# JokerYan/MS-GS

Hardware: AMD Instinct MI355X
Metric: Mpixels/s fwd+bwd @1080p, 1M Gaussians; fraction of HBM roofline (higher is better)
Workload: dtype f32

## Files before the change

__graft_entry__.py:

```python
import os
import subprocess
import sys

ROOT = os.path.dirname(os.path.abspath(__file__))
PKG = os.path.join(ROOT, "ms-gs_amd")


def _paths():
    for p in (ROOT, PKG, os.path.join(PKG, "host"), os.path.join(ROOT, "tests")):
        if p not in sys.path:
            sys.path.insert(0, p)


def build():
    subprocess.check_call(["make", "-C", PKG, "-j4"])
    subprocess.call(["make", "-C", PKG, "isa"], stdout=subprocess.DEVNULL, stderr=subprocess.DEVNULL)
    subprocess.check_call(["make", "-C", os.path.join(ROOT, "oracle")])
    _paths()
    import diff_gaussian_rasterization
    import gaussian_renderer
    import view_parallel
    lib = os.path.join(PKG, "lib", "libmsgs_hip.so")
    assert os.path.exists(lib), lib
    harness = os.path.join(PKG, "build", "libmsgs_sort_harness.so")
    assert os.path.exists(harness), harness
    harness = os.path.join(PKG, "build", "libmsgs_depth_sort_harness.so")
    assert os.path.exists(harness), harness
    print("built", lib)


def smoke():
    _paths()
    import torch
    assert torch.cuda.is_available(), "smoke() needs a GPU"
    import scenes
    from oracle import oracle_ctypes as oc
    from parity_utils import check_backward, check_forward, hip_render, small_scene
    torch.cuda.set_device(0)
    W, H = 160, 96
    sc, cam = small_scene(4000, W, H, seed=123, multiscale=True, scale_k=0.004 * 1920.0 / W * 0.25)
    st = dict(filter_small=True, filter_large=True, fade_size=0.0)
    bg = torch.tensor([0.1, 0.2, 0.3])
    dL = scenes.grad_seed(W, H, 123)
    out, pc, m2 = hip_render(sc, cam, st, bg, dL, device="cuda:0")
    orc = oc.rasterize(pc.seen, cam, st, bg)
    og = oc.backward(orc, dL)
    fwd = check_forward(out, orc, "smoke")
    bwd = check_backward(pc, m2, og, "smoke", flagged=orc.borderline_gaussians)
    print(f"smoke ok: visible={(out['radii'] > 0).sum().item()} fwd_maxdiff={fwd:.2e} bwd_rel={max(bwd.values()):.2e}")
# ... 7 lines not shown
```

ms-gs_amd/csrc/api.hip:

```cpp
#include "msgs_internal.h"

#include <atomic>
#include <new>

#include <cstring>

using namespace msgs;

namespace {

struct Timer {
    const msgs_timing_t* t;
    hipStream_t s;
    void begin(int k) const { if (t && t->ev[2 * k]) (void)hipEventRecord((hipEvent_t)t->ev[2 * k], s); }
    void end(int k) const { if (t && t->ev[2 * k + 1]) (void)hipEventRecord((hipEvent_t)t->ev[2 * k + 1], s); }
};

inline int check_inputs(const msgs_view_t* v, const msgs_gaussians_t* g) {
    if (!v || !g) return MSGS_ERR_INVALID_ARG;
    if (g->P < 0 || v->image_width <= 0 || v->image_height <= 0) return MSGS_ERR_INVALID_ARG;
    if (!v->bg || !v->viewmatrix || !v->projmatrix || !v->campos) return MSGS_ERR_INVALID_ARG;
    if (g->P > 0 && (!g->means3D || !g->opacities)) return MSGS_ERR_INVALID_ARG;
    if (g->raw_params) {
        if (g->raw_params != 1 && g->raw_params != 2) return MSGS_ERR_INVALID_ARG;
// ... 185 lines not shown
    ZeroJob zj1{nullptr, 0, (uint32_t*)(geom + GL.slab_hdr), (GL.occ_hdr - GL.slab_hdr) / 4 + sizeof(OccHeader) / 4 + 2 * (size_t)OCC_BUCKETS};
    const bool sort1_buckets = depth_sort_uses_buckets(P);
    const bool sort1_prezeroed = sort1_buckets ? depth_sort_zero_region(P, scratch + SL.sort, &zj1.p0, &zj1.n0)
                                               : radix_sort_zero_region(P, 0, 32, scratch + SL.sort, &zj1.p0, &zj1.n0);
    const bool occlusion = get_occlusion() != 0;
    uint32_t* heavy_list = occlusion ? (uint32_t*)(scratch + SL.heavy_list) : nullptr;
    uint32_t* heavy_count = occlusion ? (uint32_t*)(scratch + SL.heavy_count) : nullptr;
    uint32_t* heavy_blk = occlusion ? (uint32_t*)(scratch + SL.heavy_blk) : nullptr;
    tm.begin(MSGS_K_PREPROCESS);
    HIP_TRY(launch_preprocess(vp, *g, radii, pixel_sizes, geom, s, zj1, heavy_list, heavy_count, heavy_blk, g_deterministic.load() != 0));
    if (occlusion)
        HIP_TRY(launch_occlusion(vp, P, geom, heavy_list, heavy_count, heavy_blk, (OccCand*)(scratch + SL.occ_cand), s));
    tm.end(MSGS_K_PREPROCESS);
    if ((rc = debug_sync(view, s))) return rc;

    if (!blocking_sync()) sb.ensure();
    const bool polled = !blocking_sync() && sb.host != nullptr;
    const uint64_t ticket = ++sb.ticket;
    uint64_t* total_dev = (uint64_t*)(scratch + SL.total_out);
    uint64_t* status_dev = total_dev + 2;
    uint32_t* clamped_dev = (uint32_t*)(total_dev + 5);
    uint32_t* heavy_q_word = spec ? (uint32_t*)((char*)spec->buf.scratch2 + Stage2Scratch(spec->capacity).heavy_q) : nullptr;

    tm.begin(MSGS_K_DEPTH_SORT);
    if (sort1_buckets)
        HIP_TRY(depth_sort_buckets((const uint32_t*)(geom + GL.key), (uint32_t*)(geom + GL.skey), (uint32_t*)(geom + GL.order), P,
                                   scratch + SL.sort, s, sort1_prezeroed, (uint32_t*)(geom + GL.nvalid),
                                   (uint32_t*)(geom + GL.slab_hdr + DEPTH_SORT_INFO_OFFSET)));
    else
        HIP_TRY(radix_sort_pairs((uint32_t*)(geom + GL.key), nullptr, (uint32_t*)(geom + GL.skey),
                                 (uint32_t*)(geom + GL.order), P, 0, 32, scratch + SL.sort, s, sort1_prezeroed,
                                 (uint32_t*)(geom + GL.nvalid)));
    tm.end(MSGS_K_DEPTH_SORT);
    if ((rc = debug_sync(view, s))) return rc;
    tm.begin(MSGS_K_SCAN);
    HIP_TRY(exclusive_scan_u32((const uint32_t*)(geom + GL.tiles), (const uint32_t*)(geom + GL.order),
                               (uint32_t*)(geom + GL.offs), P, (uint64_t*)(scratch + SL.scan_partials), total_dev, s,
                               status_dev, polled ? sb.dev : nullptr, ticket,
                               (const uint32_t*)(geom + GL.nvalid), spec ? clamped_dev : nullptr,
                               spec ? (uint64_t)spec->capacity : 0, (const uint32_t*)(geom + GL.occ_hdr), heavy_q_word, nullptr,
                               vp.cell_sx >= 0 ? TILE_COUNT_MASK : 0xFFFFFFFFu,
                               vp.cell_sx >= 0 && slab_wanted(view, g) ? (uint32_t*)(geom + GL.offs_b) : nullptr,
                               &reinterpret_cast<SlabHeader*>(geom + GL.slab_hdr)->pad[0]));
    tm.end(MSGS_K_SCAN);
    pend.active = true;
    pend.polled = polled;
    pend.stream = s;
    pend.ticket = ticket;
    pend.host = sb.host;
    pend.status_dev = status_dev;
    if (spec)
        spec->launched_rc = forward_stage2_impl(view, g, geom_v, geom_bytes, spec->capacity, spec->buf, timing, stream,
                                                clamped_dev, polled ? sb.dev : nullptr, ticket);
    return MSGS_OK;
}

int forward_stage1_wait(PendingCount& pend, int64_t* num_instances_host) {
    *num_instances_host = 0;
    if (!pend.active) { t_last_info = 0; for (int k = 0; k < 4; ++k) t_last_feedback[k] = 0; return MSGS_OK; }
    pend.active = false;
    hipStream_t s = pend.stream;
    uint64_t host_status[3] = {0, 0, 0};
    if (pend.polled) {
        volatile uint64_t* hv = pend.host;
        const uint64_t ticket = pend.ticket;
        uint64_t spins = 0;
// ... 1296 lines not shown
```

ms-gs_amd/csrc/msgs_internal.h:

```cpp
#pragma once
#include <hip/hip_runtime.h>
#include <stdint.h>
#include <cmath>
#include <type_traits>
#include "../../include/msgs.h"

namespace msgs {

constexpr int TILE = MSGS_TILE;
constexpr int WAVE = 64;

struct __attribute__((aligned(16))) GaussRec { float4 r0, r1, r2; };

struct __attribute__((aligned(32))) BinRec { float4 q0, q1; };

#if defined(MSGS_GRAD_REC_F32)
typedef float grad_acc_t;
constexpr int GRAD_REC_FLOATS = 12;
#else
typedef double grad_acc_t;
constexpr int GRAD_REC_FLOATS = 10;
#endif
constexpr uint32_t TILE_ORDER_MAGIC = 0x4C505431u;
constexpr size_t GRAD_REC_BYTES = sizeof(grad_acc_t) * GRAD_REC_FLOATS;
// ... 122 lines not shown
static_assert(DEPTH_BIN_LO + DEPTH_BINS - 1 == (0x7F7FFFFFu >> DEPTH_BIN_SHIFT), "the top bin is the one of FLT_MAX");
constexpr int DEPTH_BUCKETS = 255;
constexpr int DEPTH_LDS_THREADS = 1024;
constexpr int DEPTH_LDS_ITEMS = 8;
constexpr int DEPTH_LDS_CAP = DEPTH_LDS_THREADS * DEPTH_LDS_ITEMS;
constexpr int64_t DEPTH_BUCKET_MAX_P = 1'500'000;
constexpr size_t DEPTH_SORT_INFO_OFFSET = 64;

__host__ __device__ inline uint32_t depth_bin(uint32_t key) {
    uint32_t b = key >> DEPTH_BIN_SHIFT;
    b = b < DEPTH_BIN_LO ? DEPTH_BIN_LO : b;
    b -= DEPTH_BIN_LO;
    return b < (uint32_t)DEPTH_BINS ? b : (uint32_t)DEPTH_BINS - 1u;
}

constexpr int DEPTH_HIST_KEYS = 32768;
constexpr int DEPTH_HIST_MAX_BLOCKS = 64;
constexpr int64_t DEPTH_BUCKET_HARD_MAX = (int64_t)DEPTH_HIST_KEYS * DEPTH_HIST_MAX_BLOCKS;
__host__ __device__ inline int depth_hist_blocks(int64_t n) {
    const int64_t b = (n + DEPTH_HIST_KEYS - 1) / DEPTH_HIST_KEYS;
    return b < 1 ? 1 : (b > DEPTH_HIST_MAX_BLOCKS ? DEPTH_HIST_MAX_BLOCKS : (int)b);
}

struct DepthSortScratch {
    size_t sort, coarse, map, bases, slices, total;
    __host__ __device__ explicit DepthSortScratch(int64_t n) {
        size_t o = 0;
        sort = o;   o = align256(o + SortScratch(n).total);
        coarse = o; o = align256(o + 4 * (size_t)DEPTH_COARSE);
        map = o;    o = align256(o + (size_t)DEPTH_BINS);
        bases = o;  o = align256(o + 4 * (size_t)(DEPTH_BUCKETS + 2 + 2));
        slices = o; o = align256(o + 2 * (size_t)DEPTH_BINS * depth_hist_blocks(n));
        total = o;
    }
    __host__ __device__ size_t zero_end() const { return coarse + 4 * (size_t)DEPTH_COARSE; }
};

struct Stage1Scratch {
    size_t sort, scan_partials, total_out, heavy_list, heavy_count, heavy_blk, occ_cand, total;
    __host__ __device__ explicit Stage1Scratch(int64_t P) {
        size_t o = 0;
        const size_t Pn = (size_t)(P > 0 ? P : 1);
        const size_t waves = 4 * ((Pn + 255) / 256);
        sort = o;          o = align256(o + DepthSortScratch(P).total);
        scan_partials = o; o = align256(o + 8 * (size_t)(scan_blocks(P > 0 ? P : 1) + 2));
        total_out = o;     o = align256(o + 64);
        heavy_list = o;    o = align256(o + 8 * 64 * waves);
        heavy_count = o;   o = align256(o + 4 * waves);
        heavy_blk = o;     o = align256(o + 2 * waves);
        occ_cand = o;      o = align256(o + sizeof(OccCand) * OCC_MAX_CAND);
        total = o;
    }
};

constexpr int DTRAV_SLOTS = 64;
struct BinningLayout {
    size_t ids, ranges, dtrav, total;
    __host__ __device__ BinningLayout(int64_t D, int64_t tiles) {
// ... 316 lines not shown
                                      const char* geom, const grad_acc_t* grad_rec, const msgs_grads_t& grads,
                                      hipStream_t s, bool textbook = false, bool depth = false,
                                      const CameraGrads* camera = nullptr);
hipError_t launch_blend_forward_literal(const ViewParams& vp, const char* geom, int P, const uint32_t* ids, const uint2* ranges,
                                        float* out_color, float* out_ps, float* out_depth, float* final_T, uint32_t* n_contrib,
                                        uint32_t* order_flag, hipStream_t s);
hipError_t launch_blend_backward_literal(const ViewParams& vp, const char* geom, int P, const uint32_t* ids, const uint2* ranges,
                                         const float* final_T, const uint32_t* n_contrib, const float* dL_dcolor, double* inst_grad,
                                         hipStream_t s, const float* dL_ddepth = nullptr,
                                         const float* dL_dalpha = nullptr);
hipError_t launch_sh_grad_from_views(int P, int n_views, int deg, const float* means3D, const float* campos,
                                     int64_t campos_stride, const float* drgb, int64_t drgb_stride, float scale,
                                     float* d_dc, float* d_rest, hipStream_t s);
hipError_t launch_mark_visible(int P, const float* means3D, const float* viewmatrix, const float* projmatrix,
                               uint8_t* present, hipStream_t s);
hipError_t radix_sort_pairs(uint32_t* keys_in, uint32_t* vals_in, uint32_t* keys_out, uint32_t* vals_out,
                            int64_t n, int begin_bit, int end_bit, char* scratch ,
                            hipStream_t s, bool pre_zeroed = false, uint32_t* n_valid_dev = nullptr,
                            const uint32_t* n_dev = nullptr, bool keys16 = false);
bool radix_sort_keys16_ok(int64_t n, int begin_bit, int end_bit);
bool radix_sort_zero_region(int64_t n, int begin_bit, int end_bit, char* scratch, uint32_t** ptr, size_t* words);
bool radix_sort_supports_device_count(int64_t n, int begin_bit, int end_bit);

hipError_t depth_sort_buckets(const uint32_t* keys_in, uint32_t* keys_out, uint32_t* vals_out, int64_t n,
                              char* scratch , hipStream_t s, bool pre_zeroed, uint32_t* n_valid_dev,
                              uint32_t* info = nullptr);
bool depth_sort_zero_region(int64_t n, char* scratch, uint32_t** ptr, size_t* words);
bool depth_sort_uses_buckets(int64_t n);
int set_depth_sort(int mode);
int get_depth_sort();

hipError_t exclusive_scan_u32(const uint32_t* in, const uint32_t* gather, uint32_t* out, int64_t n,
                              uint64_t* partials , uint64_t* total, hipStream_t s,
                              uint64_t* status = nullptr, uint64_t* host_mapped = nullptr, uint64_t ticket = 0,
                              const uint32_t* n_ptr = nullptr, uint32_t* clamped_total = nullptr, uint64_t clamp = 0,
                              const uint32_t* extra = nullptr,
                              uint32_t* zero_word = nullptr,
                              uint32_t* overflow_flag = nullptr, uint32_t in_mask = 0xFFFFFFFFu, uint32_t* side_out = nullptr,
                              uint32_t* side_flag = nullptr);
template <class F>
inline void with_bool(bool b, F&& f) {
    if (b) f(std::true_type{}); else f(std::false_type{});
}
hipError_t launch_zero(void* ptr, size_t bytes, hipStream_t s);
hipError_t launch_emit(const ViewParams& vp, int P, const char* geom, uint32_t* keys, uint32_t* ids,
                       int64_t D, hipStream_t s, ZeroJob zj = ZeroJob{nullptr, 0, nullptr, 0}, const uint32_t* D_dev = nullptr,
                       bool keys16 = false, uint32_t* heavy_q = nullptr, int slab = 0, const uint32_t* open_bits = nullptr,
                       int64_t density_D = 0);
hipError_t launch_slab_split(int P, char* geom, int64_t D, const uint32_t* D_dev, float fraction, uint32_t* open_bits,
// ... 140 lines not shown
```

ms-gs_amd/csrc/sort.hip:

```cpp
#include "msgs_internal.h"

#include <algorithm>
#include <atomic>
#include <cstdlib>

namespace msgs {

namespace {

__device__ __forceinline__ uint32_t wave_inclusive_scan(uint32_t v, int lane) {
#pragma unroll
    for (int off = 1; off < 64; off <<= 1) {
        const uint32_t n = (uint32_t)__shfl_up((int)v, off);
        if (lane >= off) v += n;
    }
    return v;
}

__device__ __forceinline__ uint32_t block_exclusive_scan(uint32_t v, uint32_t* s_wave , uint32_t* total) {
    const int lane = threadIdx.x & 63, w = threadIdx.x >> 6;
    const uint32_t inc = wave_inclusive_scan(v, lane);
    if (lane == 63) s_wave[w] = inc;
    __syncthreads();
    uint32_t base = 0;
// ... 51 lines not shown
    const int64_t base = (int64_t)blockIdx.x * SCAN_CHUNK + (int64_t)threadIdx.x * SCAN_ITEMS;
    uint32_t v[SCAN_ITEMS];
    if (gather) {
        uint32_t g[SCAN_ITEMS];
        scan_load_items(gather, base, n, g);
#pragma unroll
        for (int k = 0; k < SCAN_ITEMS; ++k) v[k] = base + k < n ? in[g[k]] : 0u;
        if (side_out) {
#pragma unroll
            for (int k = 0; k < SCAN_ITEMS; ++k) g[k] = v[k] >> TILE_COUNT_BITS;
            scan_store_items(side_out, base, n, g);
        }
#pragma unroll
        for (int k = 0; k < SCAN_ITEMS; ++k) v[k] &= in_mask;
        if (staged) scan_store_items(staged, base, n, v);
    } else {
        scan_load_items(in, base, n, v);
    }
    uint64_t sum = 0;
#pragma unroll
    for (int k = 0; k < SCAN_ITEMS; ++k) sum += v[k];
    const uint64_t total = block_sum_u64(sum, s_sum);
    if (threadIdx.x == 0) partials[blockIdx.x] = total;
}

__global__ __launch_bounds__(SCAN_THREADS) void scan_apply_fused_kernel(const uint32_t* in, uint32_t* out, int64_t n,
                                                                        const uint64_t* __restrict__ partials, int64_t nb,
                                                                        const uint32_t* __restrict__ n_ptr,
                                                                        uint64_t* __restrict__ total_out,
                                                                        uint64_t* __restrict__ status,
                                                                        volatile uint64_t* host, uint64_t ticket,
                                                                        uint32_t* __restrict__ clamped_total, uint64_t clamp,
                                                                        const uint32_t* __restrict__ extra,
                                                                        uint32_t* __restrict__ zero_word,
                                                                        uint32_t* __restrict__ overflow_flag) {
    __shared__ uint32_t s_wave[4];
    __shared__ uint64_t s_sum[4];
    if (n_ptr) n = (int64_t)*n_ptr;
    const int64_t chunk0 = (int64_t)blockIdx.x * SCAN_CHUNK;
    if (blockIdx.x != 0 && chunk0 >= n) return;
    const int64_t upto = blockIdx.x == 0 ? nb : (int64_t)blockIdx.x;
    uint64_t acc = 0;
    for (int64_t q = threadIdx.x; q < upto; q += SCAN_THREADS) acc += partials[q];
    const uint64_t sum = block_sum_u64(acc, s_sum);
    uint64_t base = sum;
    if (blockIdx.x == 0) {
        base = 0;
        if (threadIdx.x == 0) {
            if (total_out) *total_out = sum;
            if (zero_word) *zero_word = 0u;
            if (clamped_total) *clamped_total = (uint32_t)(sum < clamp ? sum : clamp);
            if (overflow_flag && sum > clamp) *overflow_flag = 1u;
            const uint64_t info = extra ? ((uint64_t)extra[0] | ((uint64_t)extra[1] << 32)) : 0ull;
            if (status) { status[0] = sum; status[1] = 0; status[2] = info; }
            if (host) {
                host[0] = sum;
                host[1] = 0;
                host[3] = info;
                __threadfence_system();
                host[2] = ticket;
            }
        }
        if (chunk0 >= n) return;
    }
    const int64_t tb = chunk0 + (int64_t)threadIdx.x * SCAN_ITEMS;
    uint32_t v[SCAN_ITEMS];
    scan_load_items(in, tb, n, v);
    uint32_t tsum = 0;
#pragma unroll
    for (int k = 0; k < SCAN_ITEMS; ++k) tsum += v[k];
    uint32_t total;
    uint32_t run = block_exclusive_scan(tsum, s_wave, &total) + (uint32_t)base;
#pragma unroll
    for (int k = 0; k < SCAN_ITEMS; ++k) {
        const uint32_t x = v[k];
        v[k] = run;
        run += x;
    }
    scan_store_items(out, tb, n, v);
}

struct ShiftDigit {
    int shift;
    uint32_t mask;
    __device__ __forceinline__ uint32_t operator()(uint32_t k) const { return (k >> shift) & mask; }
};
struct BucketDigit {
    const uint8_t* __restrict__ map;
    __device__ __forceinline__ uint32_t operator()(uint32_t k) const { return map[depth_bin(k)]; }
};

template <int ITEMS = SORT_ITEMS>
__device__ __forceinline__ int64_t elem_index(int64_t chunk_base, int w, int r, int lane) {
    return chunk_base + (int64_t)w * (64 * ITEMS) + r * 64 + lane;
}

template <int ITEMS, bool DROP = false, typename KeyT = uint32_t, typename Digit = ShiftDigit>
__global__ __launch_bounds__(SORT_THREADS) void radix_hist_kernel(const KeyT* __restrict__ keys, int64_t n,
                                                                  Digit dg, int64_t nblocks,
                                                                  uint32_t* __restrict__ hist,
                                                                  uint32_t* __restrict__ gsum, int gsize, int ngroups,
                                                                  const uint32_t* __restrict__ n_ptr = nullptr) {
    __shared__ uint32_t s_hist[256];
    const int64_t chunk_base = (int64_t)blockIdx.x * (SORT_THREADS * ITEMS);
    if (n_ptr) {
        n = (int64_t)*n_ptr;
        if (chunk_base >= n) return;
    }
    s_hist[threadIdx.x] = 0;
    __syncthreads();
    const int lane = threadIdx.x & 63, w = threadIdx.x >> 6;
    constexpr int KPV = 16 / (int)sizeof(KeyT);
    if (ITEMS % KPV == 0 && chunk_base + (int64_t)SORT_THREADS * ITEMS <= n) {
        const uint4* kv = reinterpret_cast<const uint4*>(keys + chunk_base);
#pragma unroll
        for (int r = 0; r < ITEMS / KPV; ++r) {
            const uint4 v = kv[r * SORT_THREADS + threadIdx.x];
            const uint32_t w4[4] = {v.x, v.y, v.z, v.w};
#pragma unroll
            for (int j = 0; j < KPV; ++j) {
                const uint32_t k = sizeof(KeyT) == 4 ? w4[j] : ((w4[j >> 1] >> ((j & 1) * 16)) & 0xFFFFu);
                if (!DROP || k != 0xFFFFFFFFu) atomicAdd(&s_hist[dg(k)], 1u);
            }
        }
    } else {
#pragma unroll
        for (int r = 0; r < ITEMS; ++r) {
            const int64_t i = elem_index<ITEMS>(chunk_base, w, r, lane);
            if (i < n) {
                const uint32_t k = (uint32_t)keys[i];
                if (!DROP || k != 0xFFFFFFFFu) atomicAdd(&s_hist[dg(k)], 1u);
            }
        }
    }
    __syncthreads();
    const uint32_t c = s_hist[threadIdx.x];
    hist[(int64_t)blockIdx.x * 256 + threadIdx.x] = c;
    if (c) atomicAdd(&gsum[(int64_t)(blockIdx.x / gsize) * 256 + threadIdx.x], c);
}

__global__ __launch_bounds__(256) void group_scan_kernel(uint32_t* __restrict__ gsum, int ngroups,
                                                         uint32_t* __restrict__ hist, int gsize, int64_t nblocks,
                                                         const uint32_t* __restrict__ n_ptr, int chunk) {
    if (n_ptr) {
        const int64_t n = (int64_t)*n_ptr;
        nblocks = (n + chunk - 1) / chunk;
        ngroups = (int)((nblocks + gsize - 1) / gsize);
        if ((int)blockIdx.x > ngroups) return;
        if (nblocks == 0) return;
    }
    const int d = threadIdx.x;
    if ((int)blockIdx.x < ngroups) {
        const int64_t first = (int64_t)blockIdx.x * gsize;
        const int rows = (int)min((int64_t)gsize, nblocks - first);
        uint32_t* q = hist + first * 256 + d;
        uint32_t run = 0;
#pragma unroll 8
        for (int k = 0; k < rows; ++k) {
            const uint32_t v = q[(int64_t)k * 256];
            q[(int64_t)k * 256] = run;
            run += v;
// ... 393 lines not shown
            if (valid && before == 0) s_cnt[w][d] = prev + (uint32_t)__popcll(peers);
        }
    }
    __syncthreads();
    uint32_t c[DEPTH_LDS_WAVES], ltot = 0;
    if (tid < 256) {
#pragma unroll
        for (int k = 0; k < DEPTH_LDS_WAVES; ++k) { c[k] = s_cnt[k][tid]; ltot += c[k]; }
    }
    const uint32_t inc = wave_inclusive_scan(ltot, lane);
    if (tid < 256 && lane == 63) s_wsum[w] = inc;
    __syncthreads();
    if (tid < 256) {
        uint32_t run = inc - ltot;
#pragma unroll
        for (int k = 0; k < 4; ++k) run += k < w ? s_wsum[k] : 0u;
#pragma unroll
        for (int k = 0; k < DEPTH_LDS_WAVES; ++k) { s_cnt[k][tid] = run; run += c[k]; }
        s_dcount[tid] = ltot;
    }
    __syncthreads();
}

__global__ __launch_bounds__(DEPTH_LDS_THREADS) void depth_lds_sort_kernel(uint32_t* keys_a, uint32_t* vals_a, uint32_t* keys_out,
                                                                           uint32_t* vals_out, const uint32_t* __restrict__ bases,
                                                                           int64_t n, uint32_t* __restrict__ info) {
    __shared__ uint32_t s_key[DEPTH_LDS_CAP], s_val[DEPTH_LDS_CAP];
    __shared__ uint32_t s_cnt[DEPTH_LDS_WAVES][256];
    __shared__ uint32_t s_wsum[4], s_dcount[256], s_run[256], s_or;
    const int tid = threadIdx.x, lane = tid & 63, w = tid >> 6;
    uint32_t lo = bases[blockIdx.x], hi = bases[blockIdx.x + 1];
    if (hi > (uint32_t)n) hi = (uint32_t)n;
    if (lo >= hi) return;
    const int64_t count = (int64_t)hi - lo;

    uint32_t key[DEPTH_LDS_ITEMS], val[DEPTH_LDS_ITEMS], rank[DEPTH_LDS_ITEMS];
    const bool fits = count <= DEPTH_LDS_CAP;
    const int R = fits ? ((int)count + DEPTH_LDS_THREADS - 1) / DEPTH_LDS_THREADS : DEPTH_LDS_ITEMS;

    if (tid == 0) s_or = 0;
    __syncthreads();
    {
        const uint32_t k0 = keys_a[lo];
        uint32_t diff = 0;
        if (fits) {
#pragma unroll
            for (int r = 0; r < DEPTH_LDS_ITEMS; ++r) {
                const int e = w * 64 * R + r * 64 + lane;
                const bool valid = r < R && e < (int)count;
                key[r] = valid ? keys_a[lo + e] : 0xFFFFFFFFu;
                val[r] = valid ? vals_a[lo + e] : 0u;
            }
#pragma unroll
            for (int r = 0; r < DEPTH_LDS_ITEMS; ++r) {
                const int e = w * 64 * R + r * 64 + lane;
                if (r < R && e < (int)count) diff |= key[r] ^ k0;
            }
        } else {
            for (int64_t i = tid; i < count; i += DEPTH_LDS_THREADS) diff |= keys_a[lo + i] ^ k0;
        }
        for (int off = 32; off > 0; off >>= 1) diff |= (uint32_t)__shfl_xor((int)diff, off);
        if (lane == 0 && diff) atomicOr(&s_or, diff);
    }
    __syncthreads();
    const int bits = 32 - __clz((int)s_or);
    int npass = (bits + 7) / 8;

    if (fits) {
        const int nloc = (int)count;
        if (npass == 0) {
#pragma unroll
            for (int r = 0; r < DEPTH_LDS_ITEMS; ++r) {
                const int e = w * 64 * R + r * 64 + lane;
                if (r < R && e < nloc) { keys_out[lo + e] = key[r]; vals_out[lo + e] = val[r]; }
            }
            return;
        }
        for (int p = 0; p < npass; ++p) {
            lds_rank(key, rank, R, nloc, 8 * p, s_cnt, s_wsum, s_dcount);
#pragma unroll
            for (int r = 0; r < DEPTH_LDS_ITEMS; ++r) {
                const int e = w * 64 * R + r * 64 + lane;
                if (r < R && e < nloc) {
                    const uint32_t lp = s_cnt[w][(key[r] >> (8 * p)) & 255u] + rank[r];
                    s_key[lp] = key[r];
                    s_val[lp] = val[r];
                }
            }
            __syncthreads();
            if (p + 1 < npass) {
#pragma unroll
                for (int r = 0; r < DEPTH_LDS_ITEMS; ++r) {
                    const int e = w * 64 * R + r * 64 + lane;
                    if (r < R && e < nloc) { key[r] = s_key[e]; val[r] = s_val[e]; }
                }
            }
        }
        for (int i = tid; i < nloc; i += DEPTH_LDS_THREADS) {
            keys_out[lo + i] = s_key[i];
            vals_out[lo + i] = s_val[i];
        }
        return;
    }

    if (tid == 0) atomicAdd(&info[1], 1u);
    if ((npass & 1) == 0) ++npass;
    for (int p = 0; p < npass; ++p) {
        const int shift = 8 * p;
        const uint32_t* src_k = (p & 1) ? keys_out : keys_a;
        const uint32_t* src_v = (p & 1) ? vals_out : vals_a;
        uint32_t* dst_k = (p & 1) ? keys_a : keys_out;
        uint32_t* dst_v = (p & 1) ? vals_a : vals_out;
        if (tid < 256) s_run[tid] = 0;
        __syncthreads();
        for (int64_t i = tid; i < count; i += DEPTH_LDS_THREADS)
            atomicAdd(&s_run[shift < 32 ? (src_k[lo + i] >> shift) & 255u : 0u], 1u);
        __syncthreads();
        if (tid == 0) {
            uint32_t run = 0;
            for (int d = 0; d < 256; ++d) { const uint32_t c = s_run[d]; s_run[d] = run; run += c; }
        }
        __syncthreads();
        for (int64_t c0 = 0; c0 < count; c0 += DEPTH_LDS_CAP) {
            const int nloc = (int)(count - c0 < DEPTH_LDS_CAP ? count - c0 : DEPTH_LDS_CAP);
// ... 2 lines not shown
            for (int r = 0; r < DEPTH_LDS_ITEMS; ++r) {
                const int e = w * 64 * R + r * 64 + lane;
                key[r] = e < nloc ? src_k[lo + c0 + e] : 0xFFFFFFFFu;
                val[r] = e < nloc ? src_v[lo + c0 + e] : 0u;
            }
            lds_rank(key, rank, R, nloc, shift, s_cnt, s_wsum, s_dcount);
#pragma unroll
            for (int r = 0; r < DEPTH_LDS_ITEMS; ++r) {
                const int e = w * 64 * R + r * 64 + lane;
                if (e < nloc) {
                    const uint32_t d = shift < 32 ? (key[r] >> shift) & 255u : 0u;
                    const uint32_t pos = s_run[d] + (s_cnt[w][d] + rank[r] - s_cnt[0][d]);
                    dst_k[lo + pos] = key[r];
                    dst_v[lo + pos] = val[r];
                }
            }
            __syncthreads();
            if (tid < 256) s_run[tid] += s_dcount[tid];
            __syncthreads();
        }
        __threadfence();
        __syncthreads();
    }
}

std::atomic<int> g_depth_sort{[] {
    const char* e = getenv("MSGS_DEPTH_SORT");
    return (e && (e[0] == '1' || e[0] == '2') && e[1] == 0) ? e[0] - '0' : 0;
}()};

template <int ITEMS>
void launch_bucket_pass(const uint32_t* src_k, uint32_t* dst_k, uint32_t* dst_v, int64_t n, const uint8_t* map, const GroupGeom& G,
                        uint32_t* hist, uint32_t* gs, hipStream_t s) {
    const dim3 grid((unsigned)G.nb), block(SORT_THREADS);
    const BucketDigit dg{map};
    hipLaunchKernelGGL((radix_hist_kernel<ITEMS, true, uint32_t, BucketDigit>), grid, block, 0, s, src_k, n, dg, G.nb, hist, gs,
                       G.gsize, G.ngroups, (const uint32_t*)nullptr);
    hipLaunchKernelGGL((radix_scatter_kernel<ITEMS, true, uint32_t, BucketDigit>), grid, block, 0, s, src_k, (const uint32_t*)nullptr,
                       dst_k, dst_v, n, dg, G.nb, (const uint32_t*)hist, (const uint32_t*)gs, G.gsize, G.ngroups, false,
                       (const uint32_t*)nullptr, (uint32_t*)nullptr);
}

}

int set_depth_sort(int mode) { return g_depth_sort.exchange(mode == 1 || mode == 2 ? mode : 0); }
int get_depth_sort() { return g_depth_sort.load(); }

bool depth_sort_uses_buckets(int64_t n) {
    const int mode = g_depth_sort.load();
    if (mode == 1 || n <= 0 || n > DEPTH_BUCKET_HARD_MAX) return false;
    return mode == 2 || n <= DEPTH_BUCKET_MAX_P;
}

bool depth_sort_zero_region(int64_t n, char* scratch, uint32_t** ptr, size_t* words) {
    const DepthSortScratch L(n);
    size_t w = 0;
    if (!radix_sort_zero_region(n, 0, 32, scratch + L.sort, ptr, &w)) return false;
    *words = (size_t)((scratch + L.zero_end()) - reinterpret_cast<char*>(*ptr)) / 4;
    return true;
}

hipError_t depth_sort_buckets(const uint32_t* keys_in, uint32_t* keys_out, uint32_t* vals_out, int64_t n, char* scratch,
                              hipStream_t s, bool pre_zeroed, uint32_t* n_valid_dev, uint32_t* info) {
    if (n <= 0) {
        if (n_valid_dev) hipLaunchKernelGGL(store_u32_kernel, dim3(1), dim3(1), 0, s, n_valid_dev, 0u);
        return hipSuccess;
    }
    const GroupGeom G(n);
    if (n > DEPTH_BUCKET_HARD_MAX) return hipErrorInvalidValue;
    const DepthSortScratch L(n);
    const SortScratch SS(n);
    char* sort = scratch + L.sort;
    uint32_t* keys_a = reinterpret_cast<uint32_t*>(sort + SS.keys_alt);
    uint32_t* vals_a = reinterpret_cast<uint32_t*>(sort + SS.vals_alt);
    uint32_t* hist = reinterpret_cast<uint32_t*>(sort + SS.hist);
    uint32_t* gsum = hist + (size_t)256 * G.nb;
    uint32_t* slices = reinterpret_cast<uint32_t*>(scratch + L.slices);
    uint32_t* coarse = reinterpret_cast<uint32_t*>(scratch + L.coarse);
    uint8_t* map = reinterpret_cast<uint8_t*>(scratch + L.map);
    uint32_t* bases = reinterpret_cast<uint32_t*>(scratch + L.bases);
    if (!info) info = bases + DEPTH_BUCKETS + 2;
    if (!pre_zeroed) {
        uint32_t* zp = nullptr;
        size_t zw = 0;
        if (!depth_sort_zero_region(n, scratch, &zp, &zw)) return hipErrorInvalidValue;
        const hipError_t e = launch_zero(zp, sizeof(uint32_t) * zw, s);
        if (e != hipSuccess) return e;
    }
    const int hb = depth_hist_blocks(n);
    hipLaunchKernelGGL(depth_hist_kernel, dim3((unsigned)hb), dim3(DEPTH_HIST_THREADS), 0, s, keys_in, n, slices, coarse);
    hipLaunchKernelGGL(depth_split_kernel, dim3(DEPTH_COARSE), dim3(256), 0, s, (const uint16_t*)slices, hb, (const uint32_t*)coarse, map,
                       bases, n_valid_dev, info);
    if (G.big) launch_bucket_pass<16>(keys_in, keys_a, vals_a, n, map, G, hist, gsum, s);
    else if (G.mid) launch_bucket_pass<8>(keys_in, keys_a, vals_a, n, map, G, hist, gsum, s);
    else launch_bucket_pass<SORT_ITEMS>(keys_in, keys_a, vals_a, n, map, G, hist, gsum, s);
    hipLaunchKernelGGL(depth_lds_sort_kernel, dim3(DEPTH_BUCKETS), dim3(DEPTH_LDS_THREADS), 0, s, keys_a, vals_a, keys_out, vals_out,
                       (const uint32_t*)bases, n, info);
    return hipGetLastError();
}

}
```

Before: 2016.

## Fuse tile-count exclusive scan into bucketed depth sort

The bucket histogram pass now also accumulates, per bucket and group, the sum of tile counts, packed with the element count into one 64-bit LDS counter. The final per-bucket LDS sort kernel derives each bucket's base offset from these sums and writes the exclusive-scan offsets, the side offsets and the published totals directly. The separate exclusive_scan_u32 pass is skipped when buckets are used. This removes a full read of tiles/order and its kernel launches, at the cost of an extra tiles read in the histogram, gathered tiles loads in the sort kernel, and more LDS and registers there.

```diff
diff --git a/__graft_entry__.py b/__graft_entry__.py
--- a/__graft_entry__.py
+++ b/__graft_entry__.py
@@ -25,6 +25,8 @@
     harness = os.path.join(PKG, "build", "libmsgs_sort_harness.so")
     assert os.path.exists(harness), harness
     harness = os.path.join(PKG, "build", "libmsgs_depth_sort_harness.so")
+    assert os.path.exists(harness), harness
+    harness = os.path.join(PKG, "build", "libmsgs_depth_sort_scan_harness.so")
     assert os.path.exists(harness), harness
     print("built", lib)
 
diff --git a/ms-gs_amd/csrc/api.hip b/ms-gs_amd/csrc/api.hip
--- a/ms-gs_amd/csrc/api.hip
+++ b/ms-gs_amd/csrc/api.hip
@@ -231,11 +231,26 @@
     uint32_t* clamped_dev = (uint32_t*)(total_dev + 5);
     uint32_t* heavy_q_word = spec ? (uint32_t*)((char*)spec->buf.scratch2 + Stage2Scratch(spec->capacity).heavy_q) : nullptr;
 
+    DepthSortScan scan;
+    scan.tiles = (const uint32_t*)(geom + GL.tiles);
+    scan.in_mask = vp.cell_sx >= 0 ? TILE_COUNT_MASK : 0xFFFFFFFFu;
+    scan.out = (uint32_t*)(geom + GL.offs);
+    scan.side_out = vp.cell_sx >= 0 && slab_wanted(view, g) ? (uint32_t*)(geom + GL.offs_b) : nullptr;
+    scan.side_flag = &reinterpret_cast<SlabHeader*>(geom + GL.slab_hdr)->pad[0];
+    scan.total = total_dev;
+    scan.status = status_dev;
+    scan.host_mapped = polled ? sb.dev : nullptr;
+    scan.ticket = ticket;
+    scan.clamped_total = spec ? clamped_dev : nullptr;
+    scan.clamp = spec ? (uint64_t)spec->capacity : 0;
+    scan.extra = (const uint32_t*)(geom + GL.occ_hdr);
+    scan.zero_word = heavy_q_word;
+
     tm.begin(MSGS_K_DEPTH_SORT);
     if (sort1_buckets)
         HIP_TRY(depth_sort_buckets((const uint32_t*)(geom + GL.key), (uint32_t*)(geom + GL.skey), (uint32_t*)(geom + GL.order), P,
                                    scratch + SL.sort, s, sort1_prezeroed, (uint32_t*)(geom + GL.nvalid),
-                                   (uint32_t*)(geom + GL.slab_hdr + DEPTH_SORT_INFO_OFFSET)));
+                                   (uint32_t*)(geom + GL.slab_hdr + DEPTH_SORT_INFO_OFFSET), &scan));
     else
         HIP_TRY(radix_sort_pairs((uint32_t*)(geom + GL.key), nullptr, (uint32_t*)(geom + GL.skey),
                                  (uint32_t*)(geom + GL.order), P, 0, 32, scratch + SL.sort, s, sort1_prezeroed,
@@ -243,14 +258,11 @@
     tm.end(MSGS_K_DEPTH_SORT);
     if ((rc = debug_sync(view, s))) return rc;
     tm.begin(MSGS_K_SCAN);
-    HIP_TRY(exclusive_scan_u32((const uint32_t*)(geom + GL.tiles), (const uint32_t*)(geom + GL.order),
-                               (uint32_t*)(geom + GL.offs), P, (uint64_t*)(scratch + SL.scan_partials), total_dev, s,
-                               status_dev, polled ? sb.dev : nullptr, ticket,
-                               (const uint32_t*)(geom + GL.nvalid), spec ? clamped_dev : nullptr,
-                               spec ? (uint64_t)spec->capacity : 0, (const uint32_t*)(geom + GL.occ_hdr), heavy_q_word, nullptr,
-                               vp.cell_sx >= 0 ? TILE_COUNT_MASK : 0xFFFFFFFFu,
-                               vp.cell_sx >= 0 && slab_wanted(view, g) ? (uint32_t*)(geom + GL.offs_b) : nullptr,
-                               &reinterpret_cast<SlabHeader*>(geom + GL.slab_hdr)->pad[0]));
+    if (!sort1_buckets)
+        HIP_TRY(exclusive_scan_u32(scan.tiles, (const uint32_t*)(geom + GL.order), scan.out, P,
+                                   (uint64_t*)(scratch + SL.scan_partials), scan.total, s, scan.status, scan.host_mapped, scan.ticket,
+                                   (const uint32_t*)(geom + GL.nvalid), scan.clamped_total, scan.clamp, scan.extra, scan.zero_word,
+                                   nullptr, scan.in_mask, scan.side_out, scan.side_flag));
     tm.end(MSGS_K_SCAN);
     pend.active = true;
     pend.polled = polled;
diff --git a/ms-gs_amd/csrc/msgs_internal.h b/ms-gs_amd/csrc/msgs_internal.h
--- a/ms-gs_amd/csrc/msgs_internal.h
+++ b/ms-gs_amd/csrc/msgs_internal.h
@@ -168,18 +168,24 @@
     return b < 1 ? 1 : (b > DEPTH_HIST_MAX_BLOCKS ? DEPTH_HIST_MAX_BLOCKS : (int)b);
 }
 
+constexpr int DEPTH_TSUM_ROWS = 32;
+
 struct DepthSortScratch {
-    size_t sort, coarse, map, bases, slices, total;
+    size_t sort, coarse, tsum, map, bases, slices, total;
+    int tsum_rows;
     __host__ __device__ explicit DepthSortScratch(int64_t n) {
         size_t o = 0;
+        const int g = SortGeom(n).ngroups;
+        tsum_rows = g < DEPTH_TSUM_ROWS ? g : DEPTH_TSUM_ROWS;
         sort = o;   o = align256(o + SortScratch(n).total);
         coarse = o; o = align256(o + 4 * (size_t)DEPTH_COARSE);
+        tsum = o;   o = align256(o + 8 * (size_t)256 * DEPTH_TSUM_ROWS);
         map = o;    o = align256(o + (size_t)DEPTH_BINS);
         bases = o;  o = align256(o + 4 * (size_t)(DEPTH_BUCKETS + 2 + 2));
         slices = o; o = align256(o + 2 * (size_t)DEPTH_BINS * depth_hist_blocks(n));
         total = o;
     }
-    __host__ __device__ size_t zero_end() const { return coarse + 4 * (size_t)DEPTH_COARSE; }
+    __host__ __device__ size_t zero_end() const { return tsum + 8 * (size_t)256 * tsum_rows; }
 };
 
 struct Stage1Scratch {
@@ -542,9 +548,24 @@
 bool radix_sort_zero_region(int64_t n, int begin_bit, int end_bit, char* scratch, uint32_t** ptr, size_t* words);
 bool radix_sort_supports_device_count(int64_t n, int begin_bit, int end_bit);
 
+struct DepthSortScan {
+    const uint32_t* tiles;
+    uint32_t in_mask;
+    uint32_t* out;
+    uint32_t* side_out;
+    uint32_t* side_flag;
+    uint64_t* total;
+    uint64_t* status;
+    uint64_t* host_mapped;
+    uint64_t ticket;
+    uint32_t* clamped_total;
+    uint64_t clamp;
+    const uint32_t* extra;
+    uint32_t* zero_word;
+};
 hipError_t depth_sort_buckets(const uint32_t* keys_in, uint32_t* keys_out, uint32_t* vals_out, int64_t n,
                               char* scratch , hipStream_t s, bool pre_zeroed, uint32_t* n_valid_dev,
-                              uint32_t* info = nullptr);
+                              uint32_t* info = nullptr, const DepthSortScan* scan = nullptr);
 bool depth_sort_zero_region(int64_t n, char* scratch, uint32_t** ptr, size_t* words);
 bool depth_sort_uses_buckets(int64_t n);
 int set_depth_sort(int mode);
diff --git a/ms-gs_amd/csrc/sort.hip b/ms-gs_amd/csrc/sort.hip
--- a/ms-gs_amd/csrc/sort.hip
+++ b/ms-gs_amd/csrc/sort.hip
@@ -97,6 +97,27 @@
     for (int k = 0; k < SCAN_ITEMS; ++k) sum += v[k];
     const uint64_t total = block_sum_u64(sum, s_sum);
     if (threadIdx.x == 0) partials[blockIdx.x] = total;
+}
+
+__device__ __forceinline__ void publish_scan_total(uint64_t sum, uint64_t* __restrict__ total_out, uint64_t* __restrict__ status,
+                                                   volatile uint64_t* host, uint64_t ticket, uint32_t* __restrict__ clamped_total,
+                                                   uint64_t clamp, const uint32_t* __restrict__ extra, uint32_t* __restrict__ zero_word,
+                                                   uint32_t* __restrict__ overflow_flag, uint32_t* __restrict__ side_flag,
+                                                   uint32_t side_value) {
+    if (total_out) *total_out = sum;
+    if (zero_word) *zero_word = 0u;
+    if (clamped_total) *clamped_total = (uint32_t)(sum < clamp ? sum : clamp);
+    if (overflow_flag && sum > clamp) *overflow_flag = 1u;
+    const uint64_t info = extra ? ((uint64_t)extra[0] | ((uint64_t)extra[1] << 32)) : 0ull;
+    if (status) { status[0] = sum; status[1] = 0; status[2] = info; }
+    if (host) {
+        host[0] = sum;
+        host[1] = 0;
+        host[3] = info;
+        __threadfence_system();
+        host[2] = ticket;
+    }
+    if (side_flag) *side_flag = side_value;
 }
 
 __global__ __launch_bounds__(SCAN_THREADS) void scan_apply_fused_kernel(const uint32_t* in, uint32_t* out, int64_t n,
@@ -121,21 +142,8 @@
     uint64_t base = sum;
     if (blockIdx.x == 0) {
         base = 0;
-        if (threadIdx.x == 0) {
-            if (total_out) *total_out = sum;
-            if (zero_word) *zero_word = 0u;
-            if (clamped_total) *clamped_total = (uint32_t)(sum < clamp ? sum : clamp);
-            if (overflow_flag && sum > clamp) *overflow_flag = 1u;
-            const uint64_t info = extra ? ((uint64_t)extra[0] | ((uint64_t)extra[1] << 32)) : 0ull;
-            if (status) { status[0] = sum; status[1] = 0; status[2] = info; }
-            if (host) {
-                host[0] = sum;
-                host[1] = 0;
-                host[3] = info;
-                __threadfence_system();
-                host[2] = ticket;
-            }
-        }
+        if (threadIdx.x == 0)
+            publish_scan_total(sum, total_out, status, host, ticket, clamped_total, clamp, extra, zero_word, overflow_flag, nullptr, 0u);
         if (chunk0 >= n) return;
     }
     const int64_t tb = chunk0 + (int64_t)threadIdx.x * SCAN_ITEMS;
@@ -156,12 +164,22 @@
 }
 
 struct ShiftDigit {
+    static constexpr bool sums = false;
     int shift;
     uint32_t mask;
     __device__ __forceinline__ uint32_t operator()(uint32_t k) const { return (k >> shift) & mask; }
 };
 struct BucketDigit {
+    static constexpr bool sums = false;
     const uint8_t* __restrict__ map;
+    __device__ __forceinline__ uint32_t operator()(uint32_t k) const { return map[depth_bin(k)]; }
+};
+struct BucketDigitSums {
+    static constexpr bool sums = true;
+    const uint8_t* __restrict__ map;
+    const uint32_t* __restrict__ tiles;
+    uint32_t in_mask;
+    unsigned long long* __restrict__ tsum;
     __device__ __forceinline__ uint32_t operator()(uint32_t k) const { return map[depth_bin(k)]; }
 };
 
@@ -176,26 +194,40 @@
                                                                   uint32_t* __restrict__ hist,
                                                                   uint32_t* __restrict__ gsum, int gsize, int ngroups,
                                                                   const uint32_t* __restrict__ n_ptr = nullptr) {
-    __shared__ uint32_t s_hist[256];
+    __shared__ uint32_t s_hist[Digit::sums ? 1 : 256];
+    __shared__ unsigned long long s_both[Digit::sums ? 256 : 1];
+    constexpr int BOTH_SHIFT = 48;
+    static_assert(SORT_THREADS * ITEMS <= 4096, "count and sum share a 64-bit counter");
     const int64_t chunk_base = (int64_t)blockIdx.x * (SORT_THREADS * ITEMS);
     if (n_ptr) {
         n = (int64_t)*n_ptr;
         if (chunk_base >= n) return;
     }
-    s_hist[threadIdx.x] = 0;
+    if constexpr (Digit::sums) s_both[threadIdx.x] = 0ull;
+    else s_hist[threadIdx.x] = 0;
     __syncthreads();
     const int lane = threadIdx.x & 63, w = threadIdx.x >> 6;
     constexpr int KPV = 16 / (int)sizeof(KeyT);
-    if (ITEMS % KPV == 0 && chunk_base + (int64_t)SORT_THREADS * ITEMS <= n) {
+    bool vec = ITEMS % KPV == 0 && chunk_base + (int64_t)SORT_THREADS * ITEMS <= n;
+    if constexpr (Digit::sums) vec = vec && sizeof(KeyT) == 4 && (reinterpret_cast<uintptr_t>(dg.tiles + chunk_base) & 15) == 0;
+    if (vec) {
         const uint4* kv = reinterpret_cast<const uint4*>(keys + chunk_base);
 #pragma unroll
         for (int r = 0; r < ITEMS / KPV; ++r) {
             const uint4 v = kv[r * SORT_THREADS + threadIdx.x];
             const uint32_t w4[4] = {v.x, v.y, v.z, v.w};
+            uint32_t t4[4] = {0u, 0u, 0u, 0u};
+            if constexpr (Digit::sums) {
+                const uint4 t = reinterpret_cast<const uint4*>(dg.tiles + chunk_base)[r * SORT_THREADS + threadIdx.x];
+                t4[0] = t.x; t4[1] = t.y; t4[2] = t.z; t4[3] = t.w;
+            }
 #pragma unroll
             for (int j = 0; j < KPV; ++j) {
                 const uint32_t k = sizeof(KeyT) == 4 ? w4[j] : ((w4[j >> 1] >> ((j & 1) * 16)) & 0xFFFFu);
-                if (!DROP || k != 0xFFFFFFFFu) atomicAdd(&s_hist[dg(k)], 1u);
+                if (!DROP || k != 0xFFFFFFFFu) {
+                    if constexpr (Digit::sums) atomicAdd(&s_both[dg(k)], (1ull << BOTH_SHIFT) + (t4[j & 3] & dg.in_mask));
+                    else atomicAdd(&s_hist[dg(k)], 1u);
+                }
             }
         }
     } else {
@@ -204,14 +236,23 @@
             const int64_t i = elem_index<ITEMS>(chunk_base, w, r, lane);
             if (i < n) {
                 const uint32_t k = (uint32_t)keys[i];
-                if (!DROP || k != 0xFFFFFFFFu) atomicAdd(&s_hist[dg(k)], 1u);
-            }
-        }
-    }
-    __syncthreads();
-    const uint32_t c = s_hist[threadIdx.x];
+                if (!DROP || k != 0xFFFFFFFFu) {
+                    if constexpr (Digit::sums) atomicAdd(&s_both[dg(k)], (1ull << BOTH_SHIFT) + (dg.tiles[i] & dg.in_mask));
+                    else atomicAdd(&s_hist[dg(k)], 1u);
+                }
+            }
+        }
+    }
+    __syncthreads();
+    uint32_t c;
+    if constexpr (Digit::sums) c = (uint32_t)(s_both[threadIdx.x] >> BOTH_SHIFT);
+    else c = s_hist[threadIdx.x];
     hist[(int64_t)blockIdx.x * 256 + threadIdx.x] = c;
     if (c) atomicAdd(&gsum[(int64_t)(blockIdx.x / gsize) * 256 + threadIdx.x], c);
+    if constexpr (Digit::sums) {
+        const unsigned long long t = s_both[threadIdx.x] & ((1ull << BOTH_SHIFT) - 1ull);
+        if (t) atomicAdd(&dg.tsum[(int64_t)(blockIdx.x / gsize) * 256 + threadIdx.x], t);
+    }
 }
 
 __global__ __launch_bounds__(256) void group_scan_kernel(uint32_t* __restrict__ gsum, int ngroups,
@@ -651,19 +692,106 @@
     __syncthreads();
 }
 
+__device__ __forceinline__ uint64_t wg_sum_u64(uint64_t v, uint64_t* s_sum ) {
+    for (int off = 32; off > 0; off >>= 1)
+        v += ((uint64_t)(uint32_t)__shfl_xor((int)(uint32_t)(v >> 32), off) << 32) | (uint32_t)__shfl_xor((int)(uint32_t)v, off);
+    if ((threadIdx.x & 63) == 0) s_sum[threadIdx.x >> 6] = v;
+    __syncthreads();
+    uint64_t t = 0;
+#pragma unroll
+    for (int k = 0; k < DEPTH_LDS_WAVES; ++k) t += s_sum[k];
+    __syncthreads();
+    return t;
+}
+
+__device__ __forceinline__ uint32_t wg_exclusive_scan(uint32_t v, uint32_t* s_w ) {
+    const int lane = threadIdx.x & 63, w = threadIdx.x >> 6;
+    const uint32_t inc = wave_inclusive_scan(v, lane);
+    if (lane == 63) s_w[w] = inc;
+    __syncthreads();
+    uint32_t base = 0;
+#pragma unroll
+    for (int k = 0; k < DEPTH_LDS_WAVES; ++k) {
+        const uint32_t t = s_w[k];
+        if (k < w) base += t;
+    }
+    __syncthreads();
+    return base + inc - v;
+}
+
+__device__ __forceinline__ void lds_bucket_offsets(const DepthSortScan& sc, uint32_t base, uint32_t lo, int nloc, int R,
+                                                   uint32_t* s_c, uint32_t* s_w) {
+    const int tid = threadIdx.x;
+    uint32_t c[DEPTH_LDS_ITEMS], tsum = 0;
+#pragma unroll
+    for (int k = 0; k < DEPTH_LDS_ITEMS; ++k) {
+        const int e = tid * R + k;
+        c[k] = (k < R && e < nloc) ? s_c[e] : 0u;
+    }
+    if (sc.side_out) {
+#pragma unroll
+        for (int k = 0; k < DEPTH_LDS_ITEMS; ++k) {
+            const int e = tid * R + k;
+            if (k < R && e < nloc) sc.side_out[lo + e] = c[k] >> TILE_COUNT_BITS;
+        }
+    }
+#pragma unroll
+    for (int k = 0; k < DEPTH_LDS_ITEMS; ++k) { c[k] &= sc.in_mask; tsum += c[k]; }
+    uint32_t run = wg_exclusive_scan(tsum, s_w) + base;
+#pragma unroll
+    for (int k = 0; k < DEPTH_LDS_ITEMS; ++k) {
+        const int e = tid * R + k;
+        if (k < R && e < nloc) { s_c[e] = run; run += c[k]; }
+    }
+    __syncthreads();
+    for (int i = tid; i < nloc; i += DEPTH_LDS_THREADS) sc.out[lo + i] = s_c[i];
+}
+
+template <bool SCAN>
 __global__ __launch_bounds__(DEPTH_LDS_THREADS) void depth_lds_sort_kernel(uint32_t* keys_a, uint32_t* vals_a, uint32_t* keys_out,
                                                                            uint32_t* vals_out, const uint32_t* __restrict__ bases,
-                                                                           int64_t n, uint32_t* __restrict__ info) {
+                                                                           int64_t n, uint32_t* __restrict__ info, DepthSortScan sc,
+                                                                           const unsigned long long* __restrict__ tsum, int rows) {
     __shared__ uint32_t s_key[DEPTH_LDS_CAP], s_val[DEPTH_LDS_CAP];
     __shared__ uint32_t s_cnt[DEPTH_LDS_WAVES][256];
     __shared__ uint32_t s_wsum[4], s_dcount[256], s_run[256], s_or;
+    __shared__ uint32_t s_c[SCAN ? DEPTH_LDS_CAP : 1];
+    __shared__ uint64_t s_sum[SCAN ? DEPTH_LDS_WAVES : 1];
+    __shared__ uint32_t s_w[SCAN ? DEPTH_LDS_WAVES : 1];
     const int tid = threadIdx.x, lane = tid & 63, w = tid >> 6;
     uint32_t lo = bases[blockIdx.x], hi = bases[blockIdx.x + 1];
     if (hi > (uint32_t)n) hi = (uint32_t)n;
-    if (lo >= hi) return;
+    if (lo >= hi && (!SCAN || blockIdx.x != 0)) return;
+    constexpr int TSUM_ROUNDS = SCAN ? DEPTH_TSUM_ROWS * 256 / DEPTH_LDS_THREADS : 1;
+    static_assert(DEPTH_TSUM_ROWS * 256 % DEPTH_LDS_THREADS == 0, "whole rounds over the table");
+    unsigned long long tv[TSUM_ROUNDS];
+    if constexpr (SCAN) {
+#pragma unroll
+        for (int j = 0; j < TSUM_ROUNDS; ++j) {
+            const int q = j * DEPTH_LDS_THREADS + tid;
+            tv[j] = (q < rows * 256 && (blockIdx.x == 0 || (uint32_t)(q & 255) < blockIdx.x)) ? tsum[q] : 0ull;
+        }
+    }
+    auto counts_in_front = [&]() -> uint64_t {
+        uint64_t acc = 0;
+#pragma unroll
+        for (int j = 0; j < TSUM_ROUNDS; ++j) acc += tv[j];
+        const uint64_t sum = wg_sum_u64(acc, s_sum);
+        if (blockIdx.x != 0) return sum;
+        if (tid == 0)
+            publish_scan_total(sum, sc.total, sc.status, (volatile uint64_t*)sc.host_mapped, sc.ticket, sc.clamped_total, sc.clamp,
+                               sc.extra, sc.zero_word, nullptr, sc.side_flag, sc.side_out ? 1u : 0u);
+        return 0;
+    };
+    (void)counts_in_front;
+    if constexpr (SCAN) {
+        if (lo >= hi) { (void)counts_in_front(); return; }
+    }
+    uint64_t base = 0;
     const int64_t count = (int64_t)hi - lo;
 
     uint32_t key[DEPTH_LDS_ITEMS], val[DEPTH_LDS_ITEMS], rank[DEPTH_LDS_ITEMS];
+    uint32_t cval[SCAN ? DEPTH_LDS_ITEMS : 1];
     const bool fits = count <= DEPTH_LDS_CAP;
     const int R = fits ? ((int)count + DEPTH_LDS_THREADS - 1) / DEPTH_LDS_THREADS : DEPTH_LDS_ITEMS;
 
@@ -680,12 +808,14 @@
                 key[r] = valid ? keys_a[lo + e] : 0xFFFFFFFFu;
                 val[r] = valid ? vals_a[lo + e] : 0u;
             }
+            if constexpr (SCAN) base = counts_in_front();
 #pragma unroll
             for (int r = 0; r < DEPTH_LDS_ITEMS; ++r) {
                 const int e = w * 64 * R + r * 64 + lane;
                 if (r < R && e < (int)count) diff |= key[r] ^ k0;
             }
         } else {
+            if constexpr (SCAN) base = counts_in_front();
             for (int64_t i = tid; i < count; i += DEPTH_LDS_THREADS) diff |= keys_a[lo + i] ^ k0;
         }
         for (int off = 32; off > 0; off >>= 1) diff |= (uint32_t)__shfl_xor((int)diff, off);
@@ -701,11 +831,28 @@
 #pragma unroll
             for (int r = 0; r < DEPTH_LDS_ITEMS; ++r) {
                 const int e = w * 64 * R + r * 64 + lane;
-                if (r < R && e < nloc) { keys_out[lo + e] = key[r]; vals_out[lo + e] = val[r]; }
+                if (r < R && e < nloc) {
+                    keys_out[lo + e] = key[r];
+                    vals_out[lo + e] = val[r];
+                    if constexpr (SCAN) s_c[e] = sc.tiles[val[r]];
+                }
+            }
+            if constexpr (SCAN) {
+                __syncthreads();
+                lds_bucket_offsets(sc, (uint32_t)base, lo, nloc, R, s_c, s_w);
             }
             return;
         }
         for (int p = 0; p < npass; ++p) {
+            if constexpr (SCAN) {
+                if (p + 1 == npass) {
+#pragma unroll
+                    for (int r = 0; r < DEPTH_LDS_ITEMS; ++r) {
+                        const int e = w * 64 * R + r * 64 + lane;
+                        cval[r] = (r < R && e < nloc) ? sc.tiles[val[r]] : 0u;
+                    }
+                }
+            }
             lds_rank(key, rank, R, nloc, 8 * p, s_cnt, s_wsum, s_dcount);
 #pragma unroll
             for (int r = 0; r < DEPTH_LDS_ITEMS; ++r) {
@@ -714,6 +861,7 @@
                     const uint32_t lp = s_cnt[w][(key[r] >> (8 * p)) & 255u] + rank[r];
                     s_key[lp] = key[r];
                     s_val[lp] = val[r];
+                    if constexpr (SCAN) { if (p + 1 == npass) s_c[lp] = cval[r]; }
                 }
             }
             __syncthreads();
@@ -729,6 +877,7 @@
             keys_out[lo + i] = s_key[i];
             vals_out[lo + i] = s_val[i];
         }
+        if constexpr (SCAN) lds_bucket_offsets(sc, (uint32_t)base, lo, nloc, R, s_c, s_w);
         return;
     }
 
@@ -777,6 +926,30 @@
         __threadfence();
         __syncthreads();
     }
+    if constexpr (SCAN) {
+        uint64_t run64 = base;
+        for (int64_t c0 = 0; c0 < count; c0 += DEPTH_LDS_CAP) {
+            const int nloc = (int)(count - c0 < DEPTH_LDS_CAP ? count - c0 : DEPTH_LDS_CAP);
+            uint32_t c[DEPTH_LDS_ITEMS], tsum = 0;
+            uint64_t tsum64 = 0;
+#pragma unroll
+            for (int k = 0; k < DEPTH_LDS_ITEMS; ++k) {
+                const int e = tid * DEPTH_LDS_ITEMS + k;
+                c[k] = e < nloc ? sc.tiles[vals_out[lo + c0 + e]] : 0u;
+                if (sc.side_out && e < nloc) sc.side_out[lo + c0 + e] = c[k] >> TILE_COUNT_BITS;
+                c[k] &= sc.in_mask;
+                tsum += c[k];
+                tsum64 += c[k];
+            }
+            uint32_t run = wg_exclusive_scan(tsum, s_w) + (uint32_t)run64;
+#pragma unroll
+            for (int k = 0; k < DEPTH_LDS_ITEMS; ++k) {
+                const int e = tid * DEPTH_LDS_ITEMS + k;
+                if (e < nloc) { sc.out[lo + c0 + e] = run; run += c[k]; }
+            }
+            run64 += wg_sum_u64(tsum64, s_sum);
+        }
+    }
 }
 
 std::atomic<int> g_depth_sort{[] {
@@ -786,11 +959,17 @@
 
 template <int ITEMS>
 void launch_bucket_pass(const uint32_t* src_k, uint32_t* dst_k, uint32_t* dst_v, int64_t n, const uint8_t* map, const GroupGeom& G,
-                        uint32_t* hist, uint32_t* gs, hipStream_t s) {
+                        uint32_t* hist, uint32_t* gs, const DepthSortScan* sc, unsigned long long* tsum, hipStream_t s) {
     const dim3 grid((unsigned)G.nb), block(SORT_THREADS);
     const BucketDigit dg{map};
-    hipLaunchKernelGGL((radix_hist_kernel<ITEMS, true, uint32_t, BucketDigit>), grid, block, 0, s, src_k, n, dg, G.nb, hist, gs,
-                       G.gsize, G.ngroups, (const uint32_t*)nullptr);
+    if (sc) {
+        const BucketDigitSums dgs{map, sc->tiles, sc->in_mask, tsum};
+        hipLaunchKernelGGL((radix_hist_kernel<ITEMS, true, uint32_t, BucketDigitSums>), grid, block, 0, s, src_k, n, dgs, G.nb, hist, gs,
+                           G.gsize, G.ngroups, (const uint32_t*)nullptr);
+    } else {
+        hipLaunchKernelGGL((radix_hist_kernel<ITEMS, true, uint32_t, BucketDigit>), grid, block, 0, s, src_k, n, dg, G.nb, hist, gs,
+                           G.gsize, G.ngroups, (const uint32_t*)nullptr);
+    }
     hipLaunchKernelGGL((radix_scatter_kernel<ITEMS, true, uint32_t, BucketDigit>), grid, block, 0, s, src_k, (const uint32_t*)nullptr,
                        dst_k, dst_v, n, dg, G.nb, (const uint32_t*)hist, (const uint32_t*)gs, G.gsize, G.ngroups, false,
                        (const uint32_t*)nullptr, (uint32_t*)nullptr);
@@ -816,14 +995,20 @@
 }
 
 hipError_t depth_sort_buckets(const uint32_t* keys_in, uint32_t* keys_out, uint32_t* vals_out, int64_t n, char* scratch,
-                              hipStream_t s, bool pre_zeroed, uint32_t* n_valid_dev, uint32_t* info) {
+                              hipStream_t s, bool pre_zeroed, uint32_t* n_valid_dev, uint32_t* info, const DepthSortScan* scan) {
+    if (scan && (!scan->tiles || !scan->out)) return hipErrorInvalidValue;
     if (n <= 0) {
         if (n_valid_dev) hipLaunchKernelGGL(store_u32_kernel, dim3(1), dim3(1), 0, s, n_valid_dev, 0u);
+        if (scan)
+            return exclusive_scan_u32(scan->tiles, vals_out, scan->out, 0, nullptr, scan->total, s, scan->status, scan->host_mapped,
+                                      scan->ticket, n_valid_dev, scan->clamped_total, scan->clamp, scan->extra, scan->zero_word, nullptr,
+                                      scan->in_mask, scan->side_out, scan->side_flag);
         return hipSuccess;
     }
     const GroupGeom G(n);
     if (n > DEPTH_BUCKET_HARD_MAX) return hipErrorInvalidValue;
     const DepthSortScratch L(n);
+    if (scan && G.ngroups > L.tsum_rows) return hipErrorInvalidValue;
     const SortScratch SS(n);
     char* sort = scratch + L.sort;
     uint32_t* keys_a = reinterpret_cast<uint32_t*>(sort + SS.keys_alt);
@@ -832,6 +1017,7 @@
     uint32_t* gsum = hist + (size_t)256 * G.nb;
     uint32_t* slices = reinterpret_cast<uint32_t*>(scratch + L.slices);
     uint32_t* coarse = reinterpret_cast<uint32_t*>(scratch + L.coarse);
+    unsigned long long* tsum = reinterpret_cast<unsigned long long*>(scratch + L.tsum);
     uint8_t* map = reinterpret_cast<uint8_t*>(scratch + L.map);
     uint32_t* bases = reinterpret_cast<uint32_t*>(scratch + L.bases);
     if (!info) info = bases + DEPTH_BUCKETS + 2;
@@ -846,11 +1032,15 @@
     hipLaunchKernelGGL(depth_hist_kernel, dim3((unsigned)hb), dim3(DEPTH_HIST_THREADS), 0, s, keys_in, n, slices, coarse);
     hipLaunchKernelGGL(depth_split_kernel, dim3(DEPTH_COARSE), dim3(256), 0, s, (const uint16_t*)slices, hb, (const uint32_t*)coarse, map,
                        bases, n_valid_dev, info);
-    if (G.big) launch_bucket_pass<16>(keys_in, keys_a, vals_a, n, map, G, hist, gsum, s);
-    else if (G.mid) launch_bucket_pass<8>(keys_in, keys_a, vals_a, n, map, G, hist, gsum, s);
-    else launch_bucket_pass<SORT_ITEMS>(keys_in, keys_a, vals_a, n, map, G, hist, gsum, s);
-    hipLaunchKernelGGL(depth_lds_sort_kernel, dim3(DEPTH_BUCKETS), dim3(DEPTH_LDS_THREADS), 0, s, keys_a, vals_a, keys_out, vals_out,
-                       (const uint32_t*)bases, n, info);
+    if (G.big) launch_bucket_pass<16>(keys_in, keys_a, vals_a, n, map, G, hist, gsum, scan, tsum, s);
+    else if (G.mid) launch_bucket_pass<8>(keys_in, keys_a, vals_a, n, map, G, hist, gsum, scan, tsum, s);
+    else launch_bucket_pass<SORT_ITEMS>(keys_in, keys_a, vals_a, n, map, G, hist, gsum, scan, tsum, s);
+    if (scan)
+        hipLaunchKernelGGL(depth_lds_sort_kernel<true>, dim3(DEPTH_BUCKETS), dim3(DEPTH_LDS_THREADS), 0, s, keys_a, vals_a, keys_out,
+                           vals_out, (const uint32_t*)bases, n, info, *scan, (const unsigned long long*)tsum, G.ngroups);
+    else
+        hipLaunchKernelGGL(depth_lds_sort_kernel<false>, dim3(DEPTH_BUCKETS), dim3(DEPTH_LDS_THREADS), 0, s, keys_a, vals_a, keys_out,
+                           vals_out, (const uint32_t*)bases, n, info, DepthSortScan{}, (const unsigned long long*)nullptr, 0);
     return hipGetLastError();
 }
 
```

After: 2033, median of 6. No clear change (+0.8%).
